# carlosmwh1985/BspAtom

Measured on AMD Instinct MI355X. Metric: l-channel eigensolves/sec at N_bsp=4096 fp64, higher is better.
Workload: dtype f64; 1 GPU; Hydrogen Coulomb l=0..127, N_bsp=4096, k=9, KIND_GRID=0 rb=800 (BASELINE configs[3]); `value` = weak scaling: 128 l-channels per GPU, 128 in total; channels_total=128, eigenvector_owner_rank=0, collective_calls=0, launched_by=python

## Files before the change

### bspatom_amd/csrc/capi.hip

```cpp
#include <atomic>
#include <new>
#include "capi_internal.h"

using namespace bsp;

namespace bsp {
static std::atomic<int> g_process_device{-1};
int process_device() { return g_process_device.load(); }
int process_device_check(int device)
{
    const int cur = g_process_device.load();
    if (cur >= 0 && cur != device) {
        fprintf(stderr, "bspatom: this process already works on device %d; use one process per GPU (device %d refused)\n", cur, device);
        return BSP_ERR_UNSUPPORTED;
    }
    return BSP_OK;
}
void process_device_latch(int device) { int expect = -1; g_process_device.compare_exchange_strong(expect, device); }
}

namespace {
struct OptName { const char *name; const char *env; int Options::*field; };
const OptName OPT_TABLE[] = {
    {"sb2st_version", "BSP_SB2ST_VERSION", &Options::sb2st_version},
// ... 5 lines not shown
    {"sb2st_diag", "BSP_SB2ST_DIAG", &Options::sb2st_diag},
    {"sb2st_force_abort", "BSP_SB2ST_FORCE_ABORT", &Options::sb2st_force_abort},
    {"sy2sb_groups", "BSP_SY2SB_GROUPS", &Options::sy2sb_groups},
    {"sy2sb_lookahead", "BSP_SY2SB_LOOKAHEAD", &Options::sy2sb_lookahead},
    {"sy2sb_segs", "BSP_SY2SB_SEGS", &Options::sy2sb_segs},
    {"panel_qr", "BSP_PANEL_QR", &Options::panel_qr},
    {"gemm_diag", "BSP_GEMM_DIAG", &Options::gemm_diag},
    {"bisect", "BSP_BISECT", &Options::bisect},
    {"bisect_ept", "BSP_BISECT_EPT", &Options::bisect_ept},
    {"bisect_tail", "BSP_BISECT_TAIL", &Options::bisect_tail},
    {"bisect_secant", "BSP_BISECT_SECANT", &Options::bisect_secant},
    {"no_eigvec_prefetch", "BSP_NO_EIGVEC_PREFETCH", &Options::no_eigvec_prefetch},
    {"vec_early", "BSP_VEC_EARLY", &Options::vec_early},
    {"vec_own_cu", "BSP_VEC_OWN_CU", &Options::vec_own_cu},
    {"poison_c", "BSP_POISON_C", &Options::poison_c},
    {"sb2sb_mfma", "BSP_SB2SB_MFMA", &Options::sb2sb_mfma},
    {"ktime", "BSP_KTIME", &Options::ktime},
    {"tsqr_regcap", "BSP_TSQR_REGCAP", &Options::tsqr_regcap},
    {"tsqr_max_m", "BSP_TSQR_MAX_M", &Options::tsqr_max_m},
    {"sb16_rows", "BSP_SB16_ROWS", &Options::sb16_rows},
    {"route", "BSP_ROUTE", &Options::route},
    {"cw_onediv", "BSP_CW_ONEDIV", &Options::cw_onediv},
    {"cw_items4", "BSP_CW_ITEMS4", &Options::cw_items4},
    {"cw_nw", "BSP_CW_NW", &Options::cw_nw},
    {"cw_ldspad", "BSP_CW_LDSPAD", &Options::cw_ldspad},
    {"cw_ipw", "BSP_CW_IPW", &Options::cw_ipw},
    {"cw_band8", "BSP_CW_BAND8", &Options::cw_band8},
    {"cw_split", "BSP_CW_SPLIT", &Options::cw_split},
    {"cw_diag", "BSP_CW_DIAG", &Options::cw_diag},
    {"s_overlap", "BSP_S_OVERLAP", &Options::s_overlap},
    {"cw_streams", "BSP_CW_STREAMS", &Options::cw_streams},
    {"cw_chunk_min", "BSP_CW_CHUNK_MIN", &Options::cw_chunk_min},
    {"sb8_wgs", "BSP_SB8_WGS", &Options::sb8_wgs},
    {"fused_probe", "BSP_FUSED_PROBE", &Options::fused_probe},
    {"dipole_stage_mb", "BSP_DIPOLE_STAGE_MB", &Options::dipole_stage_mb},
    {"wf_stage_mb", "BSP_WF_STAGE_MB", &Options::wf_stage_mb},
    {"tdse_stage_mb", "BSP_TDSE_STAGE_MB", &Options::tdse_stage_mb},
};
}

namespace bsp {
Options &opts()
{
    static Options o = [] {
        Options v;
        for (const OptName &t : OPT_TABLE) {
            const char *e = getenv(t.env);
            if (e) v.*(t.field) = (*e == 0) ? 1 : atoi(e);
        }
        return v;
    }();
    return o;
}

namespace {
struct KRec { int slot; hipEvent_t e0, e1; };
std::vector<KRec> g_krecs;
std::vector<hipEvent_t> g_kpool;
hipEvent_t g_kopen[KS_COUNT];
hipEvent_t kevent()
{
    hipEvent_t e = nullptr;
    if (!g_kpool.empty()) { e = g_kpool.back(); g_kpool.pop_back(); }
    else if (hipEventCreate(&e) != hipSuccess) e = nullptr;
    return e;
}
// ... 506 lines not shown
```

### bspatom_amd/csrc/common.h

```cpp
#pragma once
#include <hip/hip_runtime.h>
#include <cstdint>
#include <cstdio>
#include <cstdlib>

#define BSP_OK 0
#define BSP_ERR_HIP (-1)
#define BSP_ERR_ARG (-2)
#define BSP_ERR_BSPLVB (-3)
#define BSP_ERR_NOGPU (-4)
#define BSP_ERR_UNSUPPORTED (-5)

#define BSP_HIP(x)                                                                          \
    do {                                                                                    \
        hipError_t e_ = (x);                                                                \
        if (e_ != hipSuccess) {                                                             \
            fprintf(stderr, "bspatom: HIP error '%s' at %s:%d\n", hipGetErrorString(e_),    \
                    __FILE__, __LINE__);                                                    \
            return BSP_ERR_HIP;                                                             \
        }                                                                                   \
    } while (0)

typedef double double4_t __attribute__((ext_vector_type(4)));

// ... 4 lines not shown
struct Options {
    int sb2st_version = 0;
    int sb2st_ring = 0;
    int sb2st_margin = 3, sb2st_hyst = 2;
    int sb2st_lead = 0;
    int sb2st_check = 0;
    int sb2st_diag = 0;
    int sb2st_force_abort = 0;
    int sy2sb_groups = 2, sy2sb_lookahead = 1, sy2sb_segs = 0;
    int panel_qr = 3;
    int tsqr_max_m = 2048;
    int tsqr_regcap = 1;
    int gemm_diag = 0;
    int bisect = 3, bisect_ept = 0;
    int bisect_secant = 1;
    int bisect_tail = 1;
    int no_eigvec_prefetch = 0;
    int vec_early = 1;
    int vec_own_cu = 1;
    int sb2sb_mfma = 1;
    int sb16_rows = 1;
    int poison_c = 0;
    int route = 0;
    int fused_probe = 0;
    int cw_items4 = 1;
    int cw_nw = 1;
    int cw_streams = 2;
    int cw_chunk_min = 1024;
    int s_overlap = 1;
    int cw_diag = 0;
    int cw_split = 0;
    int cw_band8 = 1;
    int sb8_wgs = 0;
    int cw_ipw = 0;
    int cw_ldspad = 0;
    int cw_onediv = 0;
    int dipole_stage_mb = 0;
    int wf_stage_mb = 0;
    int tdse_stage_mb = 0;
    int ktime = 0;
};
Options &opts();

int process_device();
int process_device_check(int device);
void process_device_latch(int device);

enum KSlot { KS_SYR2K = 0, KS_SYMM, KS_PANEL_QR, KS_CHAIN, KS_SB2SB, KS_SB16ST, KS_BISECT, KS_STDFORM, KS_CRAWFORD, KS_OPBAND, KS_TDSE, KS_COUNT };
void ktime_begin(int slot, hipStream_t st);
void ktime_end(int slot, hipStream_t st);
struct KScope {
    int slot; hipStream_t st; bool on;
    KScope(int slot_, hipStream_t st_) : slot(slot_), st(st_), on(opts().ktime != 0) { if (on) ktime_begin(slot, st); }
    ~KScope() { if (on) ktime_end(slot, st); }
};

struct GemmDesc {
    int M, N, K, batch;
    const double *A; long sAm, sAk, bA;
    const double *B; long sBk, sBn, bB;
    double *C; long sCm, sCn, bC;
    double alpha, beta;
    int lower_only;
    int yoff;
    int ksplit;
    int kchunk;
// ... 139 lines not shown
```

### bspatom_amd/csrc/sbr2.hip

```cpp
#include "common.h"
#include <cstdio>
#include <cstdlib>

namespace bsp {
namespace {

constexpr int LD = 128;
constexpr int B1 = 64, NB1 = 16, LAG = 3;
constexpr int XLD = 65, VLD = 17;
constexpr int SB2SB_LDS = (64 * XLD + 3 * 64 * VLD + 16 * XLD + 2 * 16 * VLD + 16) * 8;

__device__ __forceinline__ double wsum64(double v)
{
    for (int m = 32; m; m >>= 1) v += __shfl_xor(v, m);
    return v;
}

__global__ __launch_bounds__(256) void sb2sb_kernel(int n, int npad, double *__restrict__ ABall, int t, int s_lo)
{
    extern __shared__ double lds[];
    double *X = lds, *V = X + 64 * XLD, *Y = V + 64 * VLD, *Z = Y + 64 * VLD, *W = Z + 64 * VLD, *T = W + 16 * XLD,
           *G = T + 16 * VLD, *tau = G + 16 * VLD;
    const int tid = threadIdx.x, lane = tid & 63, wv = tid >> 6;
    const int s = s_lo + blockIdx.x, k = t - LAG * s;
// ... 707 lines not shown
                const int c0 = k == 0 ? s : r0 - B2;
                const bool fast = (c0 & (WCOLS - 1)) <= WCOLS - 16 && (r0 & (WCOLS - 1)) <= WCOLS - 16;
                if (fast) chase_item<true>(Lw, pS, r0, c0, k, r, g, cA, cT, offD);
                else chase_item<false>(Lw, pS, r0, c0, k, r, g, cA, cT, offD);
                if (diag) { asm volatile("s_waitcnt lgkmcnt(0)" ::: "memory"); const long long t_ = (long long)__builtin_amdgcn_s_memtime(); dacc[2] += t_ - dt0; dt0 = t_; }
            }
            lds_only_barrier();
            if (diag) { const long long t_ = (long long)__builtin_amdgcn_s_memtime(); dacc[3] += t_ - dt0; dacc[4] += 1; }
        }
        __syncthreads();
        int hi = LP < n ? LP : n;
        for (int idx = tid; idx < (hi - RP) * WROWS; idx += 576) {
            const int c = RP + (idx >> 5), d = idx & 31;
            AB[(size_t)c * LD + d] = Lw[((c & (WCOLS - 1)) << 5) + d];
        }
        __syncthreads();
        if (pubp && tid == 0)
            __hip_atomic_store(pubp, ((unsigned long long)ps << 32) + (unsigned)n, __ATOMIC_RELAXED, __HIP_MEMORY_SCOPE_AGENT);
    }
#undef LW
    if (diag && blockIdx.x == 0 && lane == 0)
        for (int q = 0; q < 5; ++q) diag[wv * 5 + q] = dacc[q];
    if (stride > 1 && (npass - 1) % stride != w && npass > 0) return;
    __syncthreads();
    asm volatile("buffer_inv sc1" ::: "memory");
    double *dd = dall + (size_t)chn * npad, *ee = eall + (size_t)chn * npad;
    for (int j = tid; j < n; j += 576) {
        dd[j] = AB[(size_t)j * LD];
        ee[j] = j < n - 1 ? AB[(size_t)j * LD + 1] : 0.0;
    }
}

constexpr int NCW4 = 6, SB16R_THREADS = (NCW4 + 1) * 64;
__device__ __forceinline__ double &ldsb(double *Lw, int off) { return *reinterpret_cast<double *>(reinterpret_cast<char *>(Lw) + off); }

template <int B>
struct Rw {
    static constexpr int WR = 2 * B;
    static constexpr int WSH = B == 16 ? 5 : 4;
    static constexpr int RPW = 64 / B;
    static constexpr int NSW = 2 * RPW;
    static constexpr int MLAG = B == 16 ? 4 : 8;
    static constexpr int LP0 = B * (MLAG + 3);
    static constexpr int Z = WCOLS * WR;
    static constexpr int DUMP = Z + 128;
    static constexpr int XS = DUMP + 384;
    static constexpr int XPAR = NSW * 2 * B;
    static constexpr int MODE = XS + 2 * XPAR;
    static constexpr int LDS = (MODE + 2) * 8;
    static_assert(B == 16 || B == 8, "tile sizes of the rows kernel");
    static_assert((1 << WSH) == WR && XPAR == 256 && LP0 + B <= 128, "window layout");
};

template <int B>
__device__ __forceinline__ double rsumB(double x)
{
    x += dppd<0xB1>(x);
    x += dppd<0x4E>(x);
    x += dppd<0x141>(x);
    if (B == 16) x += dppd<0x140>(x);
    return x;
}
template <int B>
__device__ __forceinline__ void rsumBx2(double &a, double &b)
{
    a += dppd<0xB1>(a); b += dppd<0xB1>(b);
    a += dppd<0x4E>(a); b += dppd<0x4E>(b);
    a += dppd<0x141>(a); b += dppd<0x141>(b);
    if (B == 16) { a += dppd<0x140>(a); b += dppd<0x140>(b); }
}

template <int B>
__device__ __forceinline__ void next_reflector(double *Lw, const double x0, const int j, const int xw, const int hx)
{
    double nrm2 = j > 0 ? x0 * x0 : 0.0, alpha = j == 0 ? x0 : 0.0;
    rsumBx2<B>(nrm2, alpha);
// ... 64 lines not shown

template <int B>
__device__ __forceinline__ void chase4_bulge(double *Lw, const int r0, const int c0, const int j, const int xr, const int dumpi)
{
    double v[B], b[B];
#pragma unroll
    for (int i = 0; i < B; ++i) v[i] = Lw[xr + i];
    const double tq = Lw[xr + B];
    int ab = (((c0 + j) & (WCOLS - 1)) << Rw<B>::WSH) + (r0 - c0 - j);
    if (j == 0) ab = dumpi;
#pragma unroll
    for (int i = 0; i < B; ++i) b[i] = Lw[ab + i];
    double w0 = b[0], w1 = v[1] * b[1], w2 = v[2] * b[2], w3 = v[3] * b[3];
#pragma unroll
    for (int i = 4; i < B; i += 4) {
        w0 = fma(v[i], b[i], w0); w1 = fma(v[i + 1], b[i + 1], w1);
        w2 = fma(v[i + 2], b[i + 2], w2); w3 = fma(v[i + 3], b[i + 3], w3);
    }
    const double cb = tq * ((w0 + w1) + (w2 + w3));
#pragma unroll
    for (int i = 0; i < B; ++i) Lw[ab + i] = fma(-cb, v[i], b[i]);
}

__global__ void band_tail_zero_kernel(int n, int npad, int wr, double *__restrict__ ABall)
{
    double *AB = ABall + (size_t)blockIdx.x * ab_stride(npad);
    const int c_lo = n - (wr - 1) > 0 ? n - (wr - 1) : 0;
    for (int idx = threadIdx.x; idx < (npad + 1 - c_lo) * wr; idx += blockDim.x) {
        const int c = c_lo + idx / wr, d = idx % wr;
        if (c + d >= n) AB[(size_t)c * LD + d] = 0.0;
    }
}

template <int B, int PH>
__device__ __forceinline__ void mover_step(double *Lw, double *__restrict__ AB, const int n, const int npad, const int LP,
                                           const int RP, const int RPn, const int RPold, const int ps, const int lane,
                                           const unsigned long long *pollp, unsigned long long *pubp, unsigned long long &pw,
                                           unsigned long long &ptmp, Sb16Ctl *C, int *status, const bool diag, long long (&dacc)[5])
{
    constexpr int WSH = Rw<B>::WSH;
    long long ts = diag ? (long long)__builtin_amdgcn_s_memtime() : 0;
#define MV_STAMP(q) if (diag) { const long long t_ = (long long)__builtin_amdgcn_s_memtime(); dacc[q] += t_ - ts; ts = t_; }
    if (PH == 0 && pollp && ps > 0 && LP < n) {
        const int need = LP + 4 * B < n ? LP + 4 * B : n;
        const unsigned long long want = ((unsigned long long)(ps - 1) << 32) + (unsigned)need;
        if (pw < want) s16_wait(pollp, want, C, status);
        else asm volatile("buffer_inv sc1" ::: "memory");
    }
    if (B == 16) {
#pragma unroll
        for (int q = 0; q < 4; ++q) {
            const int c = LP + 4 * q, cl = c + (lane >> 4);
            const double *src = AB + (size_t)(cl < npad ? cl : npad) * LD + 2 * (lane & 15);
            double *dst = Lw + ((c & (WCOLS - 1)) << WSH);
            __builtin_amdgcn_global_load_lds((const __attribute__((address_space(1))) void *)src,
                                             (__attribute__((address_space(3))) void *)dst, 16, 0, 0);
        }
    } else {
        const int cl = LP + (lane >> 3);
        const double *src = AB + (size_t)(cl < npad ? cl : npad) * LD + 2 * (lane & 7);
        double *dst = Lw + ((LP & (WCOLS - 1)) << WSH);
        __builtin_amdgcn_global_load_lds((const __attribute__((address_space(1))) void *)src,
                                         (__attribute__((address_space(3))) void *)dst, 16, 0, 0);
    }
    if (PH == 1 && pollp) asm volatile("global_load_dwordx2 %0, %1, off sc1" : "+v"(ptmp) : "v"(pollp) : "memory");
    MV_STAMP(1)
    {
        const int md = lane & (Rw<B>::WR - 1), mh = lane >> WSH;
        const unsigned c0_ = (unsigned)(RP + mh), dumpo = (unsigned)npad * LD + 64 + lane;
#pragma unroll
        for (int i = 0; i < B * Rw<B>::WR / 64; ++i) {
            const unsigned c = c0_ + (64 / Rw<B>::WR) * i;
            const unsigned o = c < (unsigned)RPn ? c * LD + md : dumpo;
            AB[o] = Lw[((c & (WCOLS - 1)) << WSH) + md];
        }
    }
    MV_STAMP(0)
    if (B == 16) asm volatile("s_waitcnt vmcnt(48)" ::: "memory");
    else asm volatile("s_waitcnt vmcnt(24)" ::: "memory");
    MV_STAMP(2)
#undef MV_STAMP
    if (PH == 3 && pubp && lane == 0)
        __hip_atomic_store(pubp, ((unsigned long long)ps << 32) + (unsigned)RPold, __ATOMIC_RELAXED, __HIP_MEMORY_SCOPE_AGENT);
    if (PH == 3 && pollp) {
        const unsigned lo = __builtin_amdgcn_readfirstlane((unsigned)ptmp), hi = __builtin_amdgcn_readfirstlane((unsigned)(ptmp >> 32));
        pw = ((unsigned long long)hi << 32) | lo;
    }
}

template <int B>
__device__ __forceinline__ void stores_done_barrier()
{
    if (B == 16) asm volatile("s_waitcnt lgkmcnt(15)\n\ts_barrier" ::: "memory");
    else asm volatile("s_waitcnt lgkmcnt(7)\n\ts_barrier" ::: "memory");
}

template <int B, bool DIAG = false>
__global__ __launch_bounds__(SB16R_THREADS) void sbr_rows_kernel(int n, int npad, int batch, double *__restrict__ ABall,
                                                                 double *__restrict__ dall, double *__restrict__ eall,
                                                                 long long *diag, Sb16Ctl *ctl, int P, int *status, int force_abort)
{
    using W = Rw<B>;
    constexpr int WSH = W::WSH, WR = W::WR, RPW = W::RPW, NSW = W::NSW, MLAG = W::MLAG, LP0 = W::LP0;
    extern __shared__ double lds[];
    double *Lw = lds;
    __builtin_amdgcn_s_setprio(3);
    long long dacc[5] = {0, 0, 0, 0, 0}, dt0 = 0;
    const int tid = threadIdx.x, lane = tid & 63, wv = __builtin_amdgcn_readfirstlane(tid >> 6);
    const int j = lane & (B - 1), g = lane / B;
    const int grp = wv < 4 ? (wv >> 1) & 1 : wv & 1, role = wv < 4 ? wv & 1 : 2, sw = RPW * grp + g;
    const int zi = W::Z + 64 * grp + B * g, dumpi = W::DUMP + 64 * (wv % NCW4) + B * g;
    int chn = blockIdx.x, w = 0, stride = 1;
    const unsigned long long *pollp = nullptr;
    unsigned long long *pubp = nullptr;
    Sb16Ctl *C = nullptr;
    if (ctl) {
        const int blk = blockIdx.x, grp = blk / (8 * P), rr = blk % (8 * P);
        chn = grp * 8 + (rr & 7); w = rr >> 3;
        if (chn >= batch) return;
        C = ctl + chn;
        int *modep = reinterpret_cast<int *>(lds + W::MODE);
        if (tid == 0) {
            const unsigned long long xcc = (unsigned long long)(__builtin_amdgcn_s_getreg((31 << 11) | 20) & 0xfu);
            const unsigned long long mine = (0x10ull | xcc) << (8 * w);
            unsigned long long full = 0;
            for (int q = 0; q < P; ++q) full |= 0x10ull << (8 * q);
            unsigned long long v = atomicOr(&C->hs, mine) | mine;
            for (int spin = 0; !(v & (S16_COMMIT | S16_ABORT)); ++spin) {
                if (force_abort == 1) atomicCAS(&C->hs, v, v | S16_ABORT);
                else if ((v & full) == full) atomicCAS(&C->hs, v, v | S16_COMMIT);
                else if (spin > 400000) atomicCAS(&C->hs, v, v | S16_ABORT);
                else __builtin_amdgcn_s_sleep(4);
                v = __hip_atomic_load(&C->hs, __ATOMIC_RELAXED, __HIP_MEMORY_SCOPE_AGENT);
            }
            int mode;
            if (v & S16_ABORT) mode = (w == 0) ? 2 : 0;
            else {
                bool same = true;
                for (int q = 1; q < P; ++q) same = same && (((v >> (8 * q)) & 0xfu) == (v & 0xfu));
                if (force_abort == 2) same = false;
                mode = same ? 1 : ((w == 0) ? 2 : 0);
            }
            *modep = mode;
        }
        __syncthreads();
        const int mode = __builtin_amdgcn_readfirstlane(*modep);
        __syncthreads();
        if (mode == 0) return;
        if (mode == 1 && P > 1) { stride = P; pollp = &C->prog[(w + P - 1) % P]; pubp = &C->prog[w]; }
        else w = 0;
    }
    double *AB = ABall + (size_t)chn * ab_stride(npad);
    const int npass = (n - 2 + NSW - 1) / NSW;
    for (int ps = w; ps < npass; ps += stride) {
        const int s0 = ps * NSW;
        int RP = s0, LP = s0 + LP0;
        if (pollp && ps > 0) {
            if (tid == 0) {
                const int need = s0 + LP0 + B < n ? s0 + LP0 + B : n;
                s16_wait(pollp, ((unsigned long long)(ps - 1) << 32) + (unsigned)need, C, status);
            }
            __syncthreads();
            asm volatile("buffer_inv sc1" ::: "memory");
        }
        for (int idx = tid; idx < LP0 * WR; idx += SB16R_THREADS) {
            const int c = s0 + (idx >> WSH), d = idx & (WR - 1);
            Lw[((c & (WCOLS - 1)) << WSH) + d] = c + d < n ? AB[(size_t)c * LD + d] : 0.0;
        }
        __syncthreads();
        if (wv == 0 && g == 0) {
            const int hx = ((s0 & (WCOLS - 1)) << WSH) + 1 + j;
            next_reflector<B>(Lw, Lw[hx], j, W::XS, hx * 8);
        }
        const int nsteps = (n - s0 - 1 + B - 1) / B + LAG * (NSW - 1);
#define SB16R_RPN(t) \
        int RPn = s0 + NSW + B * ((t) - LAG * (NSW - 1) - 1);    \
        if (RPn > n) RPn = n; \
        if (RPn < RP) RPn = RP;
        if (wv == NCW4) {
            unsigned long long pw = 0, ptmp = 0;
            int RPold = RP;
            __syncthreads();
#define SB16R_MSTEP(PH) \
            if (t + PH < nsteps) { \
                SB16R_RPN(t + PH) \
                { int r4 = s0 + NSW + B * ((t + PH - MLAG) - LAG * (NSW - 1) - 1);       \
                  RPold = r4 > n ? n : (r4 < s0 ? s0 : r4); } \
                mover_step<B, PH>(Lw, AB, n, npad, LP + B * PH, RP, RPn, RPold, ps, lane, pollp, pubp, pw, ptmp, C, status, DIAG, dacc); \
                if (DIAG) dt0 = (long long)__builtin_amdgcn_s_memtime(); \
                RP = RPn; \
                lds_only_barrier(); \
                if (DIAG) { const long long t_ = (long long)__builtin_amdgcn_s_memtime(); dacc[3] += t_ - dt0; dacc[4] += 1; } \
            }
            for (int t = 0; t < nsteps; t += 4) {
                SB16R_MSTEP(0) SB16R_MSTEP(1) SB16R_MSTEP(2) SB16R_MSTEP(3)
                LP += 4 * B;
            }
#undef SB16R_MSTEP
            asm volatile("s_waitcnt vmcnt(0)" ::: "memory");
            LP = s0 + LP0;
        } else {
            const int s4 = s0 + sw;
            const bool live = s4 < n - 2;
            const int xs0 = W::XS + sw * 2 * B;
            if (role == 0) {
                double bt[B], v[B], tq = 0.0;
                int at[B];
                for (int i = 0; i < B; ++i) { bt[i] = 0.0; v[i] = 0.0; at[i] = 0; }
                if (sw == 0 && live && s4 + 1 < n) {
                    next_tile_addr<B, false>(s4 + 1, j, at);
#pragma unroll
                    for (int i = 0; i < B; ++i) { bt[i] = ldsb(Lw, at[i] + (WR - 1) * 8 * i); v[i] = Lw[xs0 + i]; }
                    tq = Lw[xs0 + B];
                }
                __syncthreads();
                for (int t = 0; t < nsteps; ++t) {
                    if (DIAG) dt0 = (long long)__builtin_amdgcn_s_memtime();
                    const int k4 = t - LAG * sw, r04 = s4 + 1 + B * k4;
                    const bool act = k4 >= 0 && live && r04 < n, actN = k4 >= -1 && live && r04 + B < n;
                    const int xw = xs0 + (((t + 1) & 1) << 8);
                    if (act) {
                        chase4_next<B>(Lw, bt, v, tq, at, j, xw);
                    } else if (k4 == -1 && live) {
                        const int hx = ((s4 & (WCOLS - 1)) << WSH) + 1 + j;
                        next_reflector<B>(Lw, Lw[hx], j, xw, hx * 8);
                    }
                    const bool wrapN = __builtin_amdgcn_ballot_w64(actN && ((r04 + B) & (WCOLS - 1)) > WCOLS - B) != 0;
                    if (actN) {
                        if (wrapN) next_tile_addr<B, false>(r04 + B, j, at);
                        else next_tile_addr<B, true>(r04 + B, j, at);
#pragma unroll
                        for (int i = 0; i < B; ++i) v[i] = Lw[xw + i];
                        tq = Lw[xw + B];
#pragma unroll
                        for (int i = 0; i < B; ++i) bt[i] = ldsb(Lw, at[i] + (WR - 1) * 8 * i);
                    }
                    if (DIAG) { const long long t_ = (long long)__builtin_amdgcn_s_memtime(); dacc[2] += t_ - dt0; dt0 = t_; }
                    if (__builtin_amdgcn_ballot_w64(actN) != 0) stores_done_barrier<B>();
                    else lds_only_barrier();
                    if (DIAG) { const long long t_ = (long long)__builtin_amdgcn_s_memtime(); dacc[3] += t_ - dt0; dacc[4] += 1; }
                }
            } else if (role == 1) {
                double d[B];
                int ad[B], offD[B];
                for (int i = 0; i < B; ++i) { d[i] = 0.0; ad[i] = 0; offD[i] = (i >= j ? (WR - 1) * j + i : (WR - 1) * i + j) * 8; }
                if (sw == 0 && live && s4 + 1 < n) {
                    diag_tile_addr<B, false>(s4 + 1, j, offD, ad);
#pragma unroll
                    for (int i = 0; i < B; ++i) d[i] = ldsb(Lw, ad[i]);
                }
                __syncthreads();
                for (int t = 0; t < nsteps; ++t) {
                    if (DIAG) dt0 = (long long)__builtin_amdgcn_s_memtime();
                    const int k4 = t - LAG * sw, r04 = s4 + 1 + B * k4;
                    const bool act = k4 >= 0 && live && r04 < n, actN = k4 >= -1 && live && r04 + B < n;
                    if (act) chase4_diag<B>(Lw, d, ad, j, xs0 + ((t & 1) << 8), zi, dumpi);
                    const bool wrapN = __builtin_amdgcn_ballot_w64(actN && ((r04 + B) & (WCOLS - 1)) > WCOLS - B) != 0;
                    if (actN) {
                        if (wrapN) diag_tile_addr<B, false>(r04 + B, j, offD, ad);
                        else diag_tile_addr<B, true>(r04 + B, j, offD, ad);
#pragma unroll
                        for (int i = 0; i < B; ++i) d[i] = ldsb(Lw, ad[i]);
                    }
                    if (DIAG) { const long long t_ = (long long)__builtin_amdgcn_s_memtime(); dacc[2] += t_ - dt0; dt0 = t_; }
                    if (__builtin_amdgcn_ballot_w64(actN) != 0) stores_done_barrier<B>();
                    else lds_only_barrier();
                    if (DIAG) { const long long t_ = (long long)__builtin_amdgcn_s_memtime(); dacc[3] += t_ - dt0; dacc[4] += 1; }
                }
            } else {
                __syncthreads();
                for (int t = 0; t < nsteps; ++t) {
                    if (DIAG) dt0 = (long long)__builtin_amdgcn_s_memtime();
                    const int k4 = t - LAG * sw, r04 = s4 + 1 + B * k4;
                    if (k4 > 0 && live && r04 < n) chase4_bulge<B>(Lw, r04, r04 - B, j, xs0 + ((t & 1) << 8), dumpi);
                    if (DIAG) { asm volatile("s_waitcnt lgkmcnt(0)" ::: "memory"); const long long t_ = (long long)__builtin_amdgcn_s_memtime(); dacc[2] += t_ - dt0; dt0 = t_; }
                    lds_only_barrier();
                    if (DIAG) { const long long t_ = (long long)__builtin_amdgcn_s_memtime(); dacc[3] += t_ - dt0; dacc[4] += 1; }
                }
            }
        }
        if (wv != NCW4 && nsteps > 0) {
            SB16R_RPN(nsteps - 1)
            RP = RPn;
        }
        LP += 4 * B * ((nsteps + 3) / 4);
#undef SB16R_RPN
        __syncthreads();
        int hi = LP < n ? LP : n;
        for (int idx = tid; idx < (hi - RP) * WR; idx += SB16R_THREADS) {
            const int c = RP + (idx >> WSH), d = idx & (WR - 1);
            AB[(size_t)c * LD + d] = Lw[((c & (WCOLS - 1)) << WSH) + d];
        }
        __syncthreads();
        if (pubp && tid == 0)
            __hip_atomic_store(pubp, ((unsigned long long)ps << 32) + (unsigned)n, __ATOMIC_RELAXED, __HIP_MEMORY_SCOPE_AGENT);
    }
    if (DIAG && blockIdx.x == 0 && lane == 0)
        for (int q = 0; q < 5; ++q) diag[wv * 5 + q] = dacc[q];
    if (stride > 1 && (npass - 1) % stride != w && npass > 0) return;
    __syncthreads();
    asm volatile("buffer_inv sc1" ::: "memory");
    double *dd = dall + (size_t)chn * npad, *ee = eall + (size_t)chn * npad;
    for (int jj = tid; jj < n; jj += SB16R_THREADS) {
        dd[jj] = AB[(size_t)jj * LD];
        ee[jj] = jj < n - 1 ? AB[(size_t)jj * LD + 1] : 0.0;
    }
}

}

int launch_sb2sb(int n, int npad, int batch, double *d_AB, hipStream_t st)
{
    static bool attr = false;
    if (!attr) {
        BSP_HIP(hipFuncSetAttribute(reinterpret_cast<const void *>(sb2sb_kernel), hipFuncAttributeMaxDynamicSharedMemorySize,
                                    SB2SB_LDS));
        BSP_HIP(hipFuncSetAttribute(reinterpret_cast<const void *>(sb2sb_mfma_kernel), hipFuncAttributeMaxDynamicSharedMemorySize,
                                    SB2SB2_LDS));
        attr = true;
    }
    const int mf = opts().sb2sb_mfma;
    if (opts().sb2st_diag) {
        int nb1 = 0, nb2 = 0;
        hipOccupancyMaxActiveBlocksPerMultiprocessor(&nb1, reinterpret_cast<const void *>(sb2sb_mfma_kernel), 256, SB2SB2_LDS);
        hipOccupancyMaxActiveBlocksPerMultiprocessor(&nb2, reinterpret_cast<const void *>(sb2sb_kernel), 256, SB2SB_LDS);
        fprintf(stderr, "sb2sb: workgroups per CU by the occupancy query: mfma kernel %d (LDS %d B), first kernel %d (LDS %d B)\n", nb1,
                SB2SB2_LDS, nb2, SB2SB_LDS);
    }
    const int S = (n - NB1 + NB1 - 1) / NB1;
    auto K = [n](int s) { const int m = n - (NB1 * s + NB1); return m > 0 ? (m + B1 - 1) / B1 : 0; };
    int tmax = -1;
    for (int s = 0; s < S; ++s)
        if (K(s) > 0 && K(s) - 1 + LAG * s > tmax) tmax = K(s) - 1 + LAG * s;
    for (int t = 0; t <= tmax; ++t) {
        int s_hi = t / LAG;
        if (s_hi > S - 1) s_hi = S - 1;
        if (t - LAG * s_hi >= K(s_hi)) continue;
        int s_lo = s_hi;
        while (s_lo > 0 && t - LAG * (s_lo - 1) < K(s_lo - 1)) --s_lo;
        KScope kt(KS_SB2SB, st);
        if (mf) hipLaunchKernelGGL(sb2sb_mfma_kernel, dim3(s_hi - s_lo + 1, batch), dim3(256), SB2SB2_LDS, st, n, npad, d_AB, t, s_lo);
        else hipLaunchKernelGGL(sb2sb_kernel, dim3(s_hi - s_lo + 1, batch), dim3(256), SB2SB_LDS, st, n, npad, d_AB, t, s_lo);
    }
    BSP_HIP(hipGetLastError());
    return BSP_OK;
}

int launch_sb16st(int n, int npad, int batch, double *d_AB, double *d_d, double *d_e, hipStream_t st, int *d_status, void *ctl, int hb)
{
    static bool attr = false;
    static int wg8 = 1;
    if (!attr) {
        BSP_HIP(hipFuncSetAttribute(reinterpret_cast<const void *>(sb16st_kernel), hipFuncAttributeMaxDynamicSharedMemorySize,
                                    SB16_LDS));
        BSP_HIP(hipFuncSetAttribute(reinterpret_cast<const void *>(sbr_rows_kernel<16, false>), hipFuncAttributeMaxDynamicSharedMemorySize,
                                    Rw<16>::LDS));
        BSP_HIP(hipFuncSetAttribute(reinterpret_cast<const void *>(sbr_rows_kernel<8, false>), hipFuncAttributeMaxDynamicSharedMemorySize,
                                    Rw<8>::LDS));
        BSP_HIP(hipFuncSetAttribute(reinterpret_cast<const void *>(sbr_rows_kernel<16, true>), hipFuncAttributeMaxDynamicSharedMemorySize,
                                    Rw<16>::LDS));
        BSP_HIP(hipFuncSetAttribute(reinterpret_cast<const void *>(sbr_rows_kernel<8, true>), hipFuncAttributeMaxDynamicSharedMemorySize,
                                    Rw<8>::LDS));
        int nb = 0;
        if (hipOccupancyMaxActiveBlocksPerMultiprocessor(&nb, reinterpret_cast<const void *>(sbr_rows_kernel<8, false>), SB16R_THREADS,
                                                         Rw<8>::LDS) == hipSuccess && nb >= 1) wg8 = nb > 2 ? 2 : nb;
        attr = true;
    }
    if (hb != 16 && hb != 8) return BSP_ERR_ARG;
    const bool rows = hb == 8 || opts().sb16_rows != 0;
    const int nsw = hb == 8 ? Rw<8>::NSW : NW2;
    int P;
    if (opts().sb2st_ring > 0) P = opts().sb2st_ring;
    else if (hb == 16) P = batch > 128 ? 1 : (batch > 64 ? 2 : (batch > 32 ? 4 : 8));
    else {
        int cus = 256;
        hipDeviceProp_t prop;
        int dev = 0;
        if (hipGetDevice(&dev) == hipSuccess && hipGetDeviceProperties(&prop, dev) == hipSuccess && prop.multiProcessorCount > 0)
            cus = prop.multiProcessorCount;
        const int wgs = opts().sb8_wgs > 0 && opts().sb8_wgs < wg8 ? opts().sb8_wgs : wg8;
        for (P = 8; P > 1 && ((batch + 7) / 8) * 8 * P > cus; P /= 2) {}
        if (P < 4 && opts().sb8_wgs == 0)
            for (P = 4; P > 1 && ((batch + 7) / 8) * 8 * P > cus * wgs; P /= 2) {}
        else if (opts().sb8_wgs > 0)
            for (P = 8; P > 1 && ((batch + 7) / 8) * 8 * P > cus * wgs; P /= 2) {}
    }
    if (P > 8) P = 8;
    while (P > 1 && (n - 2) / nsw < 2 * P) P /= 2;
    static Sb16Ctl *s_ctl = nullptr;
    static int cap = 0;
    Sb16Ctl *d_ctl = nullptr;
    static_assert(sizeof(Sb16Ctl) <= 112, "the caller's per-problem control block is sized for sb2st.hip's Sb8Ctl (112 bytes per channel)");
    if (P > 1 && ctl) {
        d_ctl = static_cast<Sb16Ctl *>(ctl);
        BSP_HIP(hipMemsetAsync(d_ctl, 0, (size_t)batch * sizeof(Sb16Ctl), st));
    }
    else if (P > 1) {
        if (cap < batch) {
            if (s_ctl) hipFree(s_ctl);
            BSP_HIP(hipMalloc(reinterpret_cast<void **>(&s_ctl), (size_t)batch * sizeof(Sb16Ctl)));
            cap = batch;
        }
        d_ctl = s_ctl;
        BSP_HIP(hipMemsetAsync(d_ctl, 0, (size_t)batch * sizeof(Sb16Ctl), st));
    }
    const int nblk = P > 1 ? ((batch + 7) / 8) * 8 * P : batch;
    const int fab = opts().sb2st_force_abort;
    auto launch = [&](long long *dbuf) {
        if (rows) hipLaunchKernelGGL(band_tail_zero_kernel, dim3(batch), dim3(256), 0, st, n, npad, 2 * hb, d_AB);
        if (hb == 8 && dbuf)
            hipLaunchKernelGGL((sbr_rows_kernel<8, true>), dim3(nblk), dim3(SB16R_THREADS), Rw<8>::LDS, st, n, npad, batch, d_AB, d_d, d_e, dbuf,
                               d_ctl, P, d_status, fab);
        else if (hb == 8)
            hipLaunchKernelGGL((sbr_rows_kernel<8, false>), dim3(nblk), dim3(SB16R_THREADS), Rw<8>::LDS, st, n, npad, batch, d_AB, d_d, d_e, dbuf,
                               d_ctl, P, d_status, fab);
        else if (rows && dbuf)
            hipLaunchKernelGGL((sbr_rows_kernel<16, true>), dim3(nblk), dim3(SB16R_THREADS), Rw<16>::LDS, st, n, npad, batch, d_AB, d_d, d_e, dbuf,
                               d_ctl, P, d_status, fab);
        else if (rows)
            hipLaunchKernelGGL((sbr_rows_kernel<16, false>), dim3(nblk), dim3(SB16R_THREADS), Rw<16>::LDS, st, n, npad, batch, d_AB, d_d, d_e, dbuf,
                               d_ctl, P, d_status, fab);
        else
            hipLaunchKernelGGL(sb16st_kernel, dim3(nblk), dim3(576), SB16_LDS, st, n, npad, batch, d_AB, d_d, d_e, dbuf, d_ctl, P,
                               d_status, fab);
    };
    if (opts().sb2st_diag) {
        long long *dbuf = nullptr, h[45];
        BSP_HIP(hipMalloc(reinterpret_cast<void **>(&dbuf), sizeof(h)));
        BSP_HIP(hipMemsetAsync(dbuf, 0, sizeof(h), st));
        launch(dbuf);
        const hipError_t le = hipGetLastError();
        if (le != hipSuccess) { hipFree(dbuf); BSP_HIP(le); }
        BSP_HIP(hipStreamSynchronize(st));
        BSP_HIP(hipMemcpy(h, dbuf, sizeof(h), hipMemcpyDeviceToHost));
        hipFree(dbuf);
        fprintf(stderr, "band chase, tiles of %d: %d workgroup(s) per channel, %d per CU\n", hb, P, hb == 8 ? wg8 : 1);
        for (int w = 0; w < 9; ++w) {
            const double steps = h[w * 5 + 4] > 0 ? (double)h[w * 5 + 4] : 1.0;
            fprintf(stderr, "sb16st wave %d: %lld steps; s_memtime ticks per step: chase item %.0f, rest + barrier %.0f (mover wave: columns out %.0f, block in %.0f)\n",
                    w, h[w * 5 + 4], (double)h[w * 5 + 2] / steps, (double)h[w * 5 + 3] / steps, (double)h[w * 5] / steps,
                    (double)h[w * 5 + 1] / steps);
        }
        return BSP_OK;
    }
    KScope kt(KS_SB16ST, st);
    launch(nullptr);
    BSP_HIP(hipGetLastError());
    return BSP_OK;
}

}
```

Measured before the change: 1907 eigensolves/s.

## Add phased steady-state step loop and short mover lag to B=8 band chase

Splits each pass of the B=8 rows band-to-tridiagonal kernel into a general prologue, a steady-state phase where every wave is known to be active, and a general epilogue. In the steady phase, LDS ring addresses are advanced incrementally and a precomputed wrap mask replaces per-step activity ballots and address recomputation. The mover wave can also run with a shorter write-back lag on short passes when several workgroups per channel are staggered, publishing progress earlier so the next pass can start sooner. It also adds a waves-per-EU hint and per-pass diagnostics, at the cost of more code paths, register pressure and extra template instances.

```diff
diff --git a/bspatom_amd/csrc/capi.hip b/bspatom_amd/csrc/capi.hip
--- a/bspatom_amd/csrc/capi.hip
+++ b/bspatom_amd/csrc/capi.hip
@@ -61,6 +61,8 @@
     {"cw_streams", "BSP_CW_STREAMS", &Options::cw_streams},
     {"cw_chunk_min", "BSP_CW_CHUNK_MIN", &Options::cw_chunk_min},
     {"sb8_wgs", "BSP_SB8_WGS", &Options::sb8_wgs},
+    {"sbr_phased", "BSP_SBR_PHASED", &Options::sbr_phased},
+    {"sbr_lag", "BSP_SBR_LAG", &Options::sbr_lag},
     {"fused_probe", "BSP_FUSED_PROBE", &Options::fused_probe},
     {"dipole_stage_mb", "BSP_DIPOLE_STAGE_MB", &Options::dipole_stage_mb},
     {"wf_stage_mb", "BSP_WF_STAGE_MB", &Options::wf_stage_mb},
diff --git a/bspatom_amd/csrc/common.h b/bspatom_amd/csrc/common.h
--- a/bspatom_amd/csrc/common.h
+++ b/bspatom_amd/csrc/common.h
@@ -60,6 +60,8 @@
     int cw_split = 0;
     int cw_band8 = 1;
     int sb8_wgs = 0;
+    int sbr_phased = 1;
+    int sbr_lag = 0;
     int cw_ipw = 0;
     int cw_ldspad = 0;
     int cw_onediv = 0;
diff --git a/bspatom_amd/csrc/sbr2.hip b/bspatom_amd/csrc/sbr2.hip
--- a/bspatom_amd/csrc/sbr2.hip
+++ b/bspatom_amd/csrc/sbr2.hip
@@ -763,6 +763,7 @@
 }
 
 constexpr int NCW4 = 6, SB16R_THREADS = (NCW4 + 1) * 64;
+constexpr int SBR_MLAG_SHORT = 2;
 __device__ __forceinline__ double &ldsb(double *Lw, int off) { return *reinterpret_cast<double *>(reinterpret_cast<char *>(Lw) + off); }
 
 template <int B>
@@ -773,6 +774,8 @@
     static constexpr int NSW = 2 * RPW;
     static constexpr int MLAG = B == 16 ? 4 : 8;
     static constexpr int LP0 = B * (MLAG + 3);
+    static constexpr int MLAGS = B == 16 ? MLAG : SBR_MLAG_SHORT;
+    static constexpr int STAGGER = LAG * NSW + 2 * MLAG + 5;
     static constexpr int Z = WCOLS * WR;
     static constexpr int DUMP = Z + 128;
     static constexpr int XS = DUMP + 384;
@@ -903,7 +906,7 @@
     }
 }
 
-template <int B, int PH>
+template <int B, int PH, int MLAG>
 __device__ __forceinline__ void mover_step(double *Lw, double *__restrict__ AB, const int n, const int npad, const int LP,
                                            const int RP, const int RPn, const int RPold, const int ps, const int lane,
                                            const unsigned long long *pollp, unsigned long long *pubp, unsigned long long &pw,
@@ -947,11 +950,14 @@
         }
     }
     MV_STAMP(0)
-    if (B == 16) asm volatile("s_waitcnt vmcnt(48)" ::: "memory");
-    else asm volatile("s_waitcnt vmcnt(24)" ::: "memory");
+    constexpr int OPS = (B == 16 ? 12 : 3) * MLAG;
+    constexpr bool SHORT = MLAG < Rw<B>::MLAG;
+    constexpr int NPOLL = !SHORT ? 0 : (MLAG >= 4 ? MLAG / 4 : (((PH + 3) & 3) < MLAG ? 1 : 0));
+    if (SHORT && NPOLL && pollp) asm volatile("s_waitcnt vmcnt(%0)" ::"n"(OPS + NPOLL) : "memory");
+    else asm volatile("s_waitcnt vmcnt(%0)" ::"n"(OPS) : "memory");
     MV_STAMP(2)
 #undef MV_STAMP
-    if (PH == 3 && pubp && lane == 0)
+    if ((PH == 3 || (SHORT && PH == 1)) && pubp && lane == 0)
         __hip_atomic_store(pubp, ((unsigned long long)ps << 32) + (unsigned)RPold, __ATOMIC_RELAXED, __HIP_MEMORY_SCOPE_AGENT);
     if (PH == 3 && pollp) {
         const unsigned lo = __builtin_amdgcn_readfirstlane((unsigned)ptmp), hi = __builtin_amdgcn_readfirstlane((unsigned)(ptmp >> 32));
@@ -966,13 +972,50 @@
     else asm volatile("s_waitcnt lgkmcnt(7)\n\ts_barrier" ::: "memory");
 }
 
-template <int B, bool DIAG = false>
-__global__ __launch_bounds__(SB16R_THREADS) void sbr_rows_kernel(int n, int npad, int batch, double *__restrict__ ABall,
-                                                                 double *__restrict__ dall, double *__restrict__ eall,
-                                                                 long long *diag, Sb16Ctl *ctl, int P, int *status, int force_abort)
+template <int B, bool DIAG, int MLAG>
+__device__ __forceinline__ void mover_pass(double *Lw, double *__restrict__ AB, const int n, const int npad, const int s0,
+                                           const int nsteps, const int ps, const int lane, const unsigned long long *pollp,
+                                           unsigned long long *pubp, Sb16Ctl *C, int *status, long long (&dacc)[5], long long *pd)
+{
+    constexpr int NSW = Rw<B>::NSW;
+    unsigned long long pw = 0, ptmp = 0;
+    int RP = s0, LP = s0 + B * (MLAG + 3), RPold = s0;
+    long long dt0 = 0;
+    const long long tp0 = DIAG ? (long long)__builtin_amdgcn_s_memtime() : 0, w0 = dacc[1];
+#define SB16R_MSTEP(PH) \
+    if (t + PH < nsteps) { \
+        int RPn = s0 + NSW + B * ((t + PH) - LAG * (NSW - 1) - 1);    \
+        if (RPn > n) RPn = n; \
+        if (RPn < RP) RPn = RP; \
+        { int r4 = s0 + NSW + B * ((t + PH - MLAG) - LAG * (NSW - 1) - 1);       \
+          RPold = r4 > n ? n : (r4 < s0 ? s0 : r4); } \
+        mover_step<B, PH, MLAG>(Lw, AB, n, npad, LP + B * PH, RP, RPn, RPold, ps, lane, pollp, pubp, pw, ptmp, C, status, DIAG, dacc); \
+        if (DIAG) dt0 = (long long)__builtin_amdgcn_s_memtime(); \
+        RP = RPn; \
+        lds_only_barrier(); \
+        if (DIAG) { const long long t_ = (long long)__builtin_amdgcn_s_memtime(); dacc[3] += t_ - dt0; dacc[4] += 1; } \
+    }
+    for (int t = 0; t < nsteps; t += 4) {
+        SB16R_MSTEP(0) SB16R_MSTEP(1) SB16R_MSTEP(2) SB16R_MSTEP(3)
+        LP += 4 * B;
+    }
+#undef SB16R_MSTEP
+    asm volatile("s_waitcnt vmcnt(0)" ::: "memory");
+    if (DIAG && pd && lane == 0) {
+        pd[0] = nsteps; pd[1] = (long long)__builtin_amdgcn_s_memtime() - tp0; pd[2] = dacc[1] - w0;
+    }
+}
+
+constexpr int SBR_PASSDIAG = 256;
+template <int B, bool DIAG, bool PHASED>
+__device__ __forceinline__ void sbr_rows_body(int n, int npad, int batch, double *__restrict__ ABall, double *__restrict__ dall,
+                                              double *__restrict__ eall, long long *diag, Sb16Ctl *ctl, int P, int *status,
+                                              int force_abort, int lagmode)
 {
     using W = Rw<B>;
     constexpr int WSH = W::WSH, WR = W::WR, RPW = W::RPW, NSW = W::NSW, MLAG = W::MLAG, LP0 = W::LP0;
+    constexpr int RINGB = WCOLS * WR * 8, STEPB = B * WR * 8;
+    static_assert(!PHASED || B == 8, "the phased step loop is built for tiles of 8");
     extern __shared__ double lds[];
     double *Lw = lds;
     __builtin_amdgcn_s_setprio(3);
@@ -1025,16 +1068,25 @@
     const int npass = (n - 2 + NSW - 1) / NSW;
     for (int ps = w; ps < npass; ps += stride) {
         const int s0 = ps * NSW;
-        int RP = s0, LP = s0 + LP0;
+        const int nsteps = (n - s0 - 1 + B - 1) / B + LAG * (NSW - 1);
+        const bool shortp = W::MLAGS < MLAG && (lagmode == 2 || (lagmode == 0 && stride > 1 && nsteps < stride * W::STAGGER));
+        const int lp0 = shortp ? B * (W::MLAGS + 3) : LP0;
+        int RP = s0, LP = s0 + lp0;
+        const long long tw0 = DIAG ? (long long)__builtin_amdgcn_s_memtime() : 0;
         if (pollp && ps > 0) {
             if (tid == 0) {
-                const int need = s0 + LP0 + B < n ? s0 + LP0 + B : n;
+                const int need = s0 + lp0 + B < n ? s0 + lp0 + B : n;
                 s16_wait(pollp, ((unsigned long long)(ps - 1) << 32) + (unsigned)need, C, status);
             }
             __syncthreads();
             asm volatile("buffer_inv sc1" ::: "memory");
         }
-        for (int idx = tid; idx < LP0 * WR; idx += SB16R_THREADS) {
+        long long *pd = nullptr;
+        if (DIAG && blockIdx.x == 0 && (ps - w) / stride < SBR_PASSDIAG) {
+            pd = diag + 45 + 4 * ((ps - w) / stride);
+            if (wv == NCW4 && lane == 0) pd[3] = (long long)__builtin_amdgcn_s_memtime() - tw0;
+        }
+        for (int idx = tid; idx < lp0 * WR; idx += SB16R_THREADS) {
             const int c = s0 + (idx >> WSH), d = idx & (WR - 1);
             Lw[((c & (WCOLS - 1)) << WSH) + d] = c + d < n ? AB[(size_t)c * LD + d] : 0.0;
         }
@@ -1043,37 +1095,32 @@
             const int hx = ((s0 & (WCOLS - 1)) << WSH) + 1 + j;
             next_reflector<B>(Lw, Lw[hx], j, W::XS, hx * 8);
         }
-        const int nsteps = (n - s0 - 1 + B - 1) / B + LAG * (NSW - 1);
-#define SB16R_RPN(t) \
-        int RPn = s0 + NSW + B * ((t) - LAG * (NSW - 1) - 1);    \
-        if (RPn > n) RPn = n; \
-        if (RPn < RP) RPn = RP;
         if (wv == NCW4) {
-            unsigned long long pw = 0, ptmp = 0;
-            int RPold = RP;
             __syncthreads();
-#define SB16R_MSTEP(PH) \
-            if (t + PH < nsteps) { \
-                SB16R_RPN(t + PH) \
-                { int r4 = s0 + NSW + B * ((t + PH - MLAG) - LAG * (NSW - 1) - 1);       \
-                  RPold = r4 > n ? n : (r4 < s0 ? s0 : r4); } \
-                mover_step<B, PH>(Lw, AB, n, npad, LP + B * PH, RP, RPn, RPold, ps, lane, pollp, pubp, pw, ptmp, C, status, DIAG, dacc); \
-                if (DIAG) dt0 = (long long)__builtin_amdgcn_s_memtime(); \
-                RP = RPn; \
-                lds_only_barrier(); \
-                if (DIAG) { const long long t_ = (long long)__builtin_amdgcn_s_memtime(); dacc[3] += t_ - dt0; dacc[4] += 1; } \
-            }
-            for (int t = 0; t < nsteps; t += 4) {
-                SB16R_MSTEP(0) SB16R_MSTEP(1) SB16R_MSTEP(2) SB16R_MSTEP(3)
-                LP += 4 * B;
-            }
-#undef SB16R_MSTEP
-            asm volatile("s_waitcnt vmcnt(0)" ::: "memory");
-            LP = s0 + LP0;
+            if (shortp) mover_pass<B, DIAG, W::MLAGS>(Lw, AB, n, npad, s0, nsteps, ps, lane, pollp, pubp, C, status, dacc, pd);
+            else mover_pass<B, DIAG, MLAG>(Lw, AB, n, npad, s0, nsteps, ps, lane, pollp, pubp, C, status, dacc, pd);
         } else {
             const int s4 = s0 + sw;
             const bool live = s4 < n - 2;
             const int xs0 = W::XS + sw * 2 * B;
+            const int r04b = s4 + 1 - B * LAG * sw;
+            int tA = nsteps, tB = nsteps;
+            unsigned long long wmask = 0;
+            if (PHASED) {
+                const int sw0 = RPW * grp, x = n - s0 - 1 - B - sw0 + B * LAG * sw0;
+                tA = LAG * (sw0 + RPW - 1);
+                tB = s0 + sw0 + RPW - 1 < n - 2 && x > 0 ? (x - 1) / B + 1 : 0;
+                if (tB > nsteps) tB = nsteps;
+                if (tA > nsteps) tA = nsteps;
+                if (tB < tA) tB = tA;
+                const int basep = r04b + B + WCOLS;
+                const int tw = (63 - (basep >> 3)) & 63, wr = (basep & 7) != 0;
+#pragma unroll
+                for (int q = 0; q < RPW; ++q) {
+                    const int twq = __builtin_amdgcn_readlane(tw, B * q), wrq = __builtin_amdgcn_readlane(wr, B * q);
+                    wmask |= (unsigned long long)wrq << twq;
+                }
+            }
             if (role == 0) {
                 double bt[B], v[B], tq = 0.0;
                 int at[B];
@@ -1085,9 +1132,9 @@
                     tq = Lw[xs0 + B];
                 }
                 __syncthreads();
-                for (int t = 0; t < nsteps; ++t) {
+                auto general_step = [&](const int t) {
                     if (DIAG) dt0 = (long long)__builtin_amdgcn_s_memtime();
-                    const int k4 = t - LAG * sw, r04 = s4 + 1 + B * k4;
+                    const int k4 = t - LAG * sw, r04 = r04b + B * t;
                     const bool act = k4 >= 0 && live && r04 < n, actN = k4 >= -1 && live && r04 + B < n;
                     const int xw = xs0 + (((t + 1) & 1) << 8);
                     if (act) {
@@ -1110,20 +1157,63 @@
                     if (__builtin_amdgcn_ballot_w64(actN) != 0) stores_done_barrier<B>();
                     else lds_only_barrier();
                     if (DIAG) { const long long t_ = (long long)__builtin_amdgcn_s_memtime(); dacc[3] += t_ - dt0; dacc[4] += 1; }
+                };
+                for (int t = 0; t < tA; ++t) general_step(t);
+                if (PHASED && tB > tA) {
+                    const unsigned long long wm2 = wmask | (wmask << 1) | (wmask >> 63);
+                    int a0 = ((((r04b + B * tA) & (WCOLS - 1)) << WSH) + B + j) * 8;
+                    int xw = xs0 + (((tA + 1) & 1) << 8);
+                    for (int t = tA; t < tB; ++t) {
+                        if (DIAG) dt0 = (long long)__builtin_amdgcn_s_memtime();
+                        if (!((wm2 >> (t & 63)) & 1)) {
+                            int af[B];
+#pragma unroll
+                            for (int i = 0; i < B; ++i) af[i] = a0;
+                            chase4_next<B>(Lw, bt, v, tq, af, j, xw);
+                            a0 = (a0 + STEPB) & (RINGB - 1);
+#pragma unroll
+                            for (int i = 0; i < B; ++i) v[i] = Lw[xw + i];
+                            tq = Lw[xw + B];
+#pragma unroll
+                            for (int i = 0; i < B; ++i) bt[i] = ldsb(Lw, a0 + (WR - 1) * 8 * i);
+                            asm volatile("; plain step" ::: "memory");
+                        } else {
+                            int ag[B];
+                            const int r04 = r04b + B * t;
+                            next_tile_addr<B, false>(r04, j, ag);
+                            chase4_next<B>(Lw, bt, v, tq, ag, j, xw);
+                            next_tile_addr<B, false>(r04 + B, j, ag);
+                            a0 = (a0 + STEPB) & (RINGB - 1);
+#pragma unroll
+                            for (int i = 0; i < B; ++i) v[i] = Lw[xw + i];
+                            tq = Lw[xw + B];
+#pragma unroll
+                            for (int i = 0; i < B; ++i) bt[i] = ldsb(Lw, ag[i] + (WR - 1) * 8 * i);
+                            asm volatile("; wrapping step" ::: "memory");
+                        }
+                        xw ^= 256;
+                        if (DIAG) { const long long t_ = (long long)__builtin_amdgcn_s_memtime(); dacc[2] += t_ - dt0; dt0 = t_; }
+                        stores_done_barrier<B>();
+                        if (DIAG) { const long long t_ = (long long)__builtin_amdgcn_s_memtime(); dacc[3] += t_ - dt0; dacc[4] += 1; }
+                    }
+                    next_tile_addr<B, false>(r04b + B * tB, j, at);
                 }
+                for (int t = tB; t < nsteps; ++t) general_step(t);
             } else if (role == 1) {
                 double d[B];
                 int ad[B], offD[B];
-                for (int i = 0; i < B; ++i) { d[i] = 0.0; ad[i] = 0; offD[i] = (i >= j ? (WR - 1) * j + i : (WR - 1) * i + j) * 8; }
+                int jo = j;
+                if (PHASED) asm volatile("" : "+v"(jo));
+                for (int i = 0; i < B; ++i) { d[i] = 0.0; ad[i] = 0; offD[i] = (i >= jo ? (WR - 1) * jo + i : (WR - 1) * i + jo) * 8; }
                 if (sw == 0 && live && s4 + 1 < n) {
                     diag_tile_addr<B, false>(s4 + 1, j, offD, ad);
 #pragma unroll
                     for (int i = 0; i < B; ++i) d[i] = ldsb(Lw, ad[i]);
                 }
                 __syncthreads();
-                for (int t = 0; t < nsteps; ++t) {
+                auto general_step = [&](const int t) {
                     if (DIAG) dt0 = (long long)__builtin_amdgcn_s_memtime();
-                    const int k4 = t - LAG * sw, r04 = s4 + 1 + B * k4;
+                    const int k4 = t - LAG * sw, r04 = r04b + B * t;
                     const bool act = k4 >= 0 && live && r04 < n, actN = k4 >= -1 && live && r04 + B < n;
                     if (act) chase4_diag<B>(Lw, d, ad, j, xs0 + ((t & 1) << 8), zi, dumpi);
                     const bool wrapN = __builtin_amdgcn_ballot_w64(actN && ((r04 + B) & (WCOLS - 1)) > WCOLS - B) != 0;
@@ -1137,25 +1227,64 @@
                     if (__builtin_amdgcn_ballot_w64(actN) != 0) stores_done_barrier<B>();
                     else lds_only_barrier();
                     if (DIAG) { const long long t_ = (long long)__builtin_amdgcn_s_memtime(); dacc[3] += t_ - dt0; dacc[4] += 1; }
+                };
+                for (int t = 0; t < tA; ++t) general_step(t);
+                if (PHASED && tB > tA) {
+                    int ud = (((r04b + B * tA) & (WCOLS - 1)) << WSH) * 8;
+                    int xr = xs0 + ((tA & 1) << 8);
+                    for (int t = tA; t < tB; ++t) {
+                        if (DIAG) dt0 = (long long)__builtin_amdgcn_s_memtime();
+                        chase4_diag<B>(Lw, d, ad, j, xr, zi, dumpi);
+                        ud = (ud + STEPB) & (RINGB - 1);
+                        if ((wmask >> (t & 63)) & 1) {
+                            diag_tile_addr<B, false>(r04b + B * (t + 1), j, offD, ad);
+                        } else {
+#pragma unroll
+                            for (int i = 0; i < B; ++i) ad[i] = ud + offD[i];
+                            asm volatile("; plain step" : "+v"(ad[0]), "+v"(ad[1]), "+v"(ad[2]), "+v"(ad[3]), "+v"(ad[4]), "+v"(ad[5]), "+v"(ad[6]), "+v"(ad[7]));
+                        }
+#pragma unroll
+                        for (int i = 0; i < B; ++i) d[i] = ldsb(Lw, ad[i]);
+                        xr ^= 256;
+                        if (DIAG) { const long long t_ = (long long)__builtin_amdgcn_s_memtime(); dacc[2] += t_ - dt0; dt0 = t_; }
+                        stores_done_barrier<B>();
+                        if (DIAG) { const long long t_ = (long long)__builtin_amdgcn_s_memtime(); dacc[3] += t_ - dt0; dacc[4] += 1; }
+                    }
                 }
+                for (int t = tB; t < nsteps; ++t) general_step(t);
             } else {
                 __syncthreads();
-                for (int t = 0; t < nsteps; ++t) {
+                auto general_step = [&](const int t) {
                     if (DIAG) dt0 = (long long)__builtin_amdgcn_s_memtime();
-                    const int k4 = t - LAG * sw, r04 = s4 + 1 + B * k4;
+                    const int k4 = t - LAG * sw, r04 = r04b + B * t;
                     if (k4 > 0 && live && r04 < n) chase4_bulge<B>(Lw, r04, r04 - B, j, xs0 + ((t & 1) << 8), dumpi);
                     if (DIAG) { asm volatile("s_waitcnt lgkmcnt(0)" ::: "memory"); const long long t_ = (long long)__builtin_amdgcn_s_memtime(); dacc[2] += t_ - dt0; dt0 = t_; }
                     lds_only_barrier();
                     if (DIAG) { const long long t_ = (long long)__builtin_amdgcn_s_memtime(); dacc[3] += t_ - dt0; dacc[4] += 1; }
+                };
+                const int tA2 = tA + 1 < tB ? tA + 1 : tB;
+                for (int t = 0; t < tA2; ++t) general_step(t);
+                if (PHASED && tB > tA2) {
+                    int r04 = r04b + B * tA2, xr = xs0 + ((tA2 & 1) << 8);
+                    for (int t = tA2; t < tB; ++t) {
+                        if (DIAG) dt0 = (long long)__builtin_amdgcn_s_memtime();
+                        chase4_bulge<B>(Lw, r04, r04 - B, j, xr, dumpi);
+                        r04 += B; xr ^= 256;
+                        if (DIAG) { asm volatile("s_waitcnt lgkmcnt(0)" ::: "memory"); const long long t_ = (long long)__builtin_amdgcn_s_memtime(); dacc[2] += t_ - dt0; dt0 = t_; }
+                        lds_only_barrier();
+                        if (DIAG) { const long long t_ = (long long)__builtin_amdgcn_s_memtime(); dacc[3] += t_ - dt0; dacc[4] += 1; }
+                    }
                 }
+                for (int t = tB; t < nsteps; ++t) general_step(t);
             }
         }
-        if (wv != NCW4 && nsteps > 0) {
-            SB16R_RPN(nsteps - 1)
+        if (nsteps > 0) {
+            int RPn = s0 + NSW + B * ((nsteps - 1) - LAG * (NSW - 1) - 1);
+            if (RPn > n) RPn = n;
+            if (RPn < RP) RPn = RP;
             RP = RPn;
         }
         LP += 4 * B * ((nsteps + 3) / 4);
-#undef SB16R_RPN
         __syncthreads();
         int hi = LP < n ? LP : n;
         for (int idx = tid; idx < (hi - RP) * WR; idx += SB16R_THREADS) {
@@ -1177,6 +1306,20 @@
         ee[jj] = jj < n - 1 ? AB[(size_t)jj * LD + 1] : 0.0;
     }
 }
+
+#define SBR_ROWS_ARGS int n, int npad, int batch, double *__restrict__ ABall, double *__restrict__ dall, double *__restrict__ eall, \
+                      long long *diag, Sb16Ctl *ctl, int P, int *status, int force_abort, int lagmode
+template <int B, bool DIAG = false>
+__global__ __launch_bounds__(SB16R_THREADS) __attribute__((amdgpu_waves_per_eu(B == 8 ? 4 : 2))) void sbr_rows_kernel(SBR_ROWS_ARGS)
+{
+    sbr_rows_body<B, DIAG, B == 8>(n, npad, batch, ABall, dall, eall, diag, ctl, P, status, force_abort, lagmode);
+}
+template <int B, bool DIAG = false>
+__global__ __launch_bounds__(SB16R_THREADS) __attribute__((amdgpu_waves_per_eu(B == 8 ? 4 : 2))) void sbr_rows_general_kernel(SBR_ROWS_ARGS)
+{
+    sbr_rows_body<B, DIAG, false>(n, npad, batch, ABall, dall, eall, diag, ctl, P, status, force_abort, lagmode);
+}
+#undef SBR_ROWS_ARGS
 
 }
 
@@ -1224,14 +1367,11 @@
     if (!attr) {
         BSP_HIP(hipFuncSetAttribute(reinterpret_cast<const void *>(sb16st_kernel), hipFuncAttributeMaxDynamicSharedMemorySize,
                                     SB16_LDS));
-        BSP_HIP(hipFuncSetAttribute(reinterpret_cast<const void *>(sbr_rows_kernel<16, false>), hipFuncAttributeMaxDynamicSharedMemorySize,
-                                    Rw<16>::LDS));
-        BSP_HIP(hipFuncSetAttribute(reinterpret_cast<const void *>(sbr_rows_kernel<8, false>), hipFuncAttributeMaxDynamicSharedMemorySize,
-                                    Rw<8>::LDS));
-        BSP_HIP(hipFuncSetAttribute(reinterpret_cast<const void *>(sbr_rows_kernel<16, true>), hipFuncAttributeMaxDynamicSharedMemorySize,
-                                    Rw<16>::LDS));
-        BSP_HIP(hipFuncSetAttribute(reinterpret_cast<const void *>(sbr_rows_kernel<8, true>), hipFuncAttributeMaxDynamicSharedMemorySize,
-                                    Rw<8>::LDS));
+        const void *const rk16[] = {reinterpret_cast<const void *>(sbr_rows_kernel<16, false>), reinterpret_cast<const void *>(sbr_rows_kernel<16, true>)};
+        const void *const rk8[] = {reinterpret_cast<const void *>(sbr_rows_kernel<8, false>), reinterpret_cast<const void *>(sbr_rows_kernel<8, true>),
+                                   reinterpret_cast<const void *>(sbr_rows_general_kernel<8, false>), reinterpret_cast<const void *>(sbr_rows_general_kernel<8, true>)};
+        for (const void *f : rk16) BSP_HIP(hipFuncSetAttribute(f, hipFuncAttributeMaxDynamicSharedMemorySize, Rw<16>::LDS));
+        for (const void *f : rk8) BSP_HIP(hipFuncSetAttribute(f, hipFuncAttributeMaxDynamicSharedMemorySize, Rw<8>::LDS));
         int nb = 0;
         if (hipOccupancyMaxActiveBlocksPerMultiprocessor(&nb, reinterpret_cast<const void *>(sbr_rows_kernel<8, false>), SB16R_THREADS,
                                                          Rw<8>::LDS) == hipSuccess && nb >= 1) wg8 = nb > 2 ? 2 : nb;
@@ -1277,26 +1417,30 @@
     }
     const int nblk = P > 1 ? ((batch + 7) / 8) * 8 * P : batch;
     const int fab = opts().sb2st_force_abort;
+    const bool phased = opts().sbr_phased != 0;
+    const int lagmode = opts().sbr_lag;
     auto launch = [&](long long *dbuf) {
         if (rows) hipLaunchKernelGGL(band_tail_zero_kernel, dim3(batch), dim3(256), 0, st, n, npad, 2 * hb, d_AB);
-        if (hb == 8 && dbuf)
-            hipLaunchKernelGGL((sbr_rows_kernel<8, true>), dim3(nblk), dim3(SB16R_THREADS), Rw<8>::LDS, st, n, npad, batch, d_AB, d_d, d_e, dbuf,
-                               d_ctl, P, d_status, fab);
-        else if (hb == 8)
-            hipLaunchKernelGGL((sbr_rows_kernel<8, false>), dim3(nblk), dim3(SB16R_THREADS), Rw<8>::LDS, st, n, npad, batch, d_AB, d_d, d_e, dbuf,
-                               d_ctl, P, d_status, fab);
+#define SBR_LAUNCH(K, ...) hipLaunchKernelGGL((K<__VA_ARGS__>), dim3(nblk), dim3(SB16R_THREADS), Rw<8>::LDS, st, n, npad, batch, d_AB, d_d, d_e, dbuf, \
+                                              d_ctl, P, d_status, fab, lagmode)
+        if (hb == 8 && dbuf && phased) SBR_LAUNCH(sbr_rows_kernel, 8, true);
+        else if (hb == 8 && dbuf) SBR_LAUNCH(sbr_rows_general_kernel, 8, true);
+        else if (hb == 8 && phased) SBR_LAUNCH(sbr_rows_kernel, 8, false);
+        else if (hb == 8) SBR_LAUNCH(sbr_rows_general_kernel, 8, false);
+#undef SBR_LAUNCH
         else if (rows && dbuf)
             hipLaunchKernelGGL((sbr_rows_kernel<16, true>), dim3(nblk), dim3(SB16R_THREADS), Rw<16>::LDS, st, n, npad, batch, d_AB, d_d, d_e, dbuf,
-                               d_ctl, P, d_status, fab);
+                               d_ctl, P, d_status, fab, 1);
         else if (rows)
             hipLaunchKernelGGL((sbr_rows_kernel<16, false>), dim3(nblk), dim3(SB16R_THREADS), Rw<16>::LDS, st, n, npad, batch, d_AB, d_d, d_e, dbuf,
-                               d_ctl, P, d_status, fab);
+                               d_ctl, P, d_status, fab, 1);
         else
             hipLaunchKernelGGL(sb16st_kernel, dim3(nblk), dim3(576), SB16_LDS, st, n, npad, batch, d_AB, d_d, d_e, dbuf, d_ctl, P,
                                d_status, fab);
     };
     if (opts().sb2st_diag) {
-        long long *dbuf = nullptr, h[45];
+        static long long h[45 + 4 * SBR_PASSDIAG];
+        long long *dbuf = nullptr;
         BSP_HIP(hipMalloc(reinterpret_cast<void **>(&dbuf), sizeof(h)));
         BSP_HIP(hipMemsetAsync(dbuf, 0, sizeof(h), st));
         launch(dbuf);
@@ -1312,6 +1456,12 @@
                     w, h[w * 5 + 4], (double)h[w * 5 + 2] / steps, (double)h[w * 5 + 3] / steps, (double)h[w * 5] / steps,
                     (double)h[w * 5 + 1] / steps);
         }
+        for (int q = 0; q < SBR_PASSDIAG && h[45 + 4 * q] > 0; ++q) {
+            const long long *pq = h + 45 + 4 * q;
+            const double tick = (double)pq[1] / (double)pq[0];
+            fprintf(stderr, "sb16st pass %d of workgroup 0: %lld steps, %.0f ticks per step; waited %.1f steps for its start, %.1f steps in poll check + requests\n",
+                    q, pq[0], tick, (double)pq[3] / tick, (double)pq[2] / tick);
+        }
         return BSP_OK;
     }
     KScope kt(KS_SB16ST, st);
```

New measurement: 1965 eigensolves/s, median of 6. +3.0%, better.
